# initc3/HoneyBadgerMPC

Measured on AMD Instinct MI355X. Metric: shares reconstructed/sec (batch open, n=64 t=21), higher is better.
Workload: dtype u256 (integer mod p): exact int8 x int8 -> int32 byte-split GEMM on the matrix cores; the high half of every sum folded mod p on the matrix cores too, one-word Barrett quotient

## Files before the change

### honeybadgermpc_amd/csrc/hb_mfma_fused.hip

```cpp
#include <math.h>

#include <algorithm>
#include <atomic>
#include <type_traits>

#include "hb_mm8.hpp"

namespace hb {

#include "hb_mm8_body.inc"

constexpr int FS_WAVES = 8, FS_TPW = 4;
#ifdef HB_MM8_TIMING
__device__ unsigned long long g_fs_t[256 * 8 * 8];
#define FS_T(k) do { const unsigned long long tn_ = __builtin_amdgcn_s_memtime(); tacc[k] += tn_ - tlast; tlast = tn_; } while (0)
#else
#define FS_T(k) do { } while (0)
#endif
constexpr int FS_MAXD = 24, FS_MAXC = 104;
constexpr size_t FS_LDS_LIMIT = 156 * 1024;

struct FsIdx { uint16_t z[FS_MAXD], xz[FS_MAXD], zc[FS_MAXC], xzc[FS_MAXC]; };
struct FsPick { const uint4 *cand; const uint32_t *cand_crow; int n_coef, nc; uint16_t zc[FS_MAXC]; };
struct FsSplit { uint32_t terms[FS_WAVES]; };
struct FsPack { int nm, ns; uint8_t single[8]; };
__host__ __device__ inline int fs_slot(const FsPack &pk, int i, int n_out, int &kind) {
    kind = 0;
    if (!(pk.nm | pk.ns)) return i;
    const int base = 16 * ((n_out + 15) / 16 - 1);
    int before = 0;
    for (int k = 0; k < pk.ns; k++) {
        if (pk.single[k] == i) { kind = 2; return base + 4 + (k & 3) + 8 * (k >> 2); }
        before += pk.single[k] < i;
    }
    const int pos = i - before;
    if (pos >= base) kind = 1;
    return pos;
}
static bool fs_pack_decide(int d, int n_coef, int nc, const uint8_t *small, FsPack *pk) {
    memset(pk, 0, sizeof *pk);
    const int n_out = n_coef + nc, rem = n_out - 16 * ((n_out + 15) / 16 - 1);
    if ((int64_t)d * 8 * 128 * 128 > MM8_BIAS_PACK) return false;
    if (rem <= 8) { pk->nm = rem; return true; }
    if (rem == 16) return false;
    int ns = 0;
    for (int i = n_coef - 1; i >= 0 && ns < 8; i--)
        if (small[i]) pk->single[ns++] = (uint8_t)i;
    std::reverse(pk->single, pk->single + ns);
    if (rem - ns > 4) { memset(pk, 0, sizeof *pk); return false; }
    pk->nm = rem - ns; pk->ns = ns;
    return true;
}
constexpr int FS_CAND_MAXN = 128;

__host__ __device__ inline int fs_ms_q(int d) { return (d + 1) * 64 + d * 8; }
__host__ __device__ inline size_t fs_lds_bytes(int n_rt, int nkb, int ms_d = 0) {
    return ((size_t)n_rt * 64 + (size_t)n_rt * nkb * 2 * 64 + (size_t)2 * FS_TPW * nkb * 4 * 64 + MM8_FOLD_Q + (ms_d ? fs_ms_q(ms_d) : 0)) * 16 +
           (size_t)(32 + 16 * n_rt) * 4;
}

#define FS_REDUCE(I_, F_, E_, C0_) \
    do { \
        const int i = (I_); \
        const int md = maskl[i]; \
        const bool live = chunk < n_chunks; \
        const bool cmp = live && md > 0, st = live && md < 0; \
        uint32_t ew[8]; \
        load_words<8>(ew, in_pk + (cmp ? (chunk * in_sc + (int64_t)(md - 1) * in_sl) * 8 : 0)); \
        uint64_t pw[8]; \
        { \
            const uint4 *cr = reinterpret_cast<const uint4 *>(crl + (size_t)i * 16); \
        _Pragma("unroll") \
            for (int k = 0; k < 4; k++) { \
                const uint4 c = cr[k]; \
                pw[2 * k] = (uint64_t)c.x | ((uint64_t)c.y << 32); \
                pw[2 * k + 1] = (uint64_t)c.z | ((uint64_t)c.w << 32); \
            } \
        } \
        uint32_t glo[5], ghi[5]; \
        _Pragma("unroll") \
        for (int k = 0; k < 12; k++) { \
            uint64_t gk = (uint64_t)F_(k) * k256 + (k < 7 ? pw[k] : 0ull); \
            if (k < 11) gk += (uint64_t)E_(k) * k16m; \
            if (k < 7) pw[k] = gk; \
            else { glo[k - 7] = (uint32_t)gk; ghi[k - 7] = (uint32_t)(gk >> 32); } \
        } \
        pw[0] += (uint64_t)(C0_) * u1; \
        pw[7] += (uint64_t)glo[0] * u1; \
        uint32_t hw[5]; \
        { \
            unsigned cyw = 0; \
        _Pragma("unroll") \
            for (int k = 0; k < 4; k++) hw[k] = __builtin_addc(glo[k + 1], ghi[k], cyw, &cyw); \
            hw[4] = ghi[4] + cyw; \
        } \
        v4i hb; \
        _Pragma("unroll") \
        for (int k = 0; k < 4; k++) hb[k] = (int)(hw[k] ^ 0x80808080u); \
        v4i dcol[8]; \
        _Pragma("unroll") \
        for (int eb = 0; eb < 8; eb++) \
            dcol[eb] = __builtin_amdgcn_mfma_i32_16x16x64_i8(fold_lane[eb * (MM8_FOLD_ROW / 16)], hb, v4i{0, 0, 0, 0}, 0, 0, 0); \
        _Pragma("unroll") \
        for (int k = 0; k < 8; k++) pw[k] += (uint64_t)hw[4] * bp.c384[k]; \
        _Pragma("unroll") \
        for (int k = 0; k < 8; k++) { \
            int64_t tt = (int64_t)pw[k] + (int64_t)dcol[k][0] * s1; \
            tt += (int64_t)dcol[k][1] * s256; \
            tt += (int64_t)dcol[k][2] * s64k; \
            tt += (int64_t)dcol[k][3] * s16m; \
            pw[k] = (uint64_t)tt; \
        } \
        const uint64_t tq = pw[7] + (pw[6] >> 32); \
        const uint32_t qh = (uint32_t)(((uint64_t)(uint32_t)(tq >> 16) * bp.mu) >> 46); \
        _Pragma("unroll") \
        for (int k = 0; k < 8; k++) pw[k] += (uint64_t)qh * bp.pneg[k]; \
        uint32_t ow[8]; \
        uint32_t top; \
        { \
            unsigned cy = 0; \
            ow[0] = (uint32_t)pw[0]; \
        _Pragma("unroll") \
            for (int k = 1; k < 8; k++) ow[k] = __builtin_addc((uint32_t)pw[k], (uint32_t)(pw[k - 1] >> 32), cy, &cy); \
            top = (uint32_t)(pw[7] >> 32) + cy - qh; \
        } \
        if (__builtin_amdgcn_ballot_w64(top != 0 || ow[7] >= ~bp.pneg[7]) != 0) { \
            uint32_t u[8]; \
            unsigned cy2 = 0; \
        _Pragma("unroll") \
            for (int k = 0; k < 8; k++) u[k] = __builtin_addc(ow[k], bp.pneg[k], cy2, &cy2); \
            const bool take = cy2 || top; \
        _Pragma("unroll") \
            for (int k = 0; k < 8; k++) ow[k] = take ? u[k] : ow[k]; \
        } \
        uint32_t diff = 0; \
        _Pragma("unroll") \
        for (int k = 0; k < 8; k++) diff |= ew[k] ^ ow[k]; \
        asm volatile("" : "+v"(diff), "+v"(ow[0]), "+v"(ow[1]), "+v"(ow[2]), "+v"(ow[3]), "+v"(ow[4]), "+v"(ow[5]), "+v"(ow[6]), "+v"(ow[7])); \
        const unsigned long long bad_lanes = __builtin_amdgcn_ballot_w64(cmp && diff); \
        if (bad_lanes) { \
            const uint32_t bits16 = (uint32_t)((bad_lanes | (bad_lanes >> 16) | (bad_lanes >> 32) | (bad_lanes >> 48)) & 0xffffull); \
            if (lane == 0) { \
                const int64_t tile_base = chunk - n; \
                const int32_t cmin = (int32_t)tile_base + __builtin_ctz(bits16); \
                if (*reinterpret_cast<volatile int32_t *>(mismatch) == 0) atomicOr(mismatch, 1); \
                if (first_bad && *reinterpret_cast<volatile int32_t *>(first_bad) > cmin) atomicMin(first_bad, cmin); \
                if (bad_map) atomicOr(bad_map + (tile_base >> 5), bits16 << (tile_base & 31)); \
            } \
        } \
        const int64_t oidx = chunk * out_sc + (int64_t)(-md - 1) * out_sl; \
        if (st && oidx < out_count) store_words<8>(out_pk + oidx * 8, ow); \
    } while (0)

template <int NKB, int PK, bool MSC>
__global__ __launch_bounds__(64 * FS_WAVES, 2) void k_mm8f(const int4 *__restrict__ a8, const uint32_t *__restrict__ crowd, const v4i *__restrict__ foldg,
                                                          const uint32_t *__restrict__ KT, const PrescaleParams PP,
                                                          const uint32_t *__restrict__ in_pk, int64_t in_sc, int64_t in_sl, const int32_t *__restrict__ in_rows,
                                                          int64_t in_count, int d, const int32_t *__restrict__ rowmode,
                                                          uint32_t *__restrict__ out_pk, int64_t out_sc, int64_t out_sl, int64_t out_count,
                                                          int32_t *__restrict__ mismatch, int32_t *__restrict__ first_bad, uint32_t *__restrict__ bad_map,
                                                          int n_out, int n_rt, int64_t n_chunks, int64_t n_units, BarrettParams bp, const FsDone done, const FsPick pick,
                                                          const FsSplit split, const v4i *__restrict__ MS) {
    constexpr bool PACKED = PK != 0;
    const int n_slots = PACKED ? 16 * n_rt : n_out;
    constexpr int NT = 64 * FS_WAVES, NL = 9, NW = 8;
    extern __shared__ uint4 fs_lds[];
    const int lane = threadIdx.x & 63, wave = __builtin_amdgcn_readfirstlane(threadIdx.x >> 6);
    const int n = lane & 15, g = lane >> 4;
    uint32_t *crl = reinterpret_cast<uint32_t *>(fs_lds);
    int4 *abuf = reinterpret_cast<int4 *>(fs_lds + n_rt * 64);
    uint4 *xbuf = fs_lds + n_rt * 64 + n_rt * NKB * 2 * 64;
    constexpr int bufsz = FS_TPW * NKB * 4 * 64;
    int32_t *rowl = reinterpret_cast<int32_t *>(xbuf + 2 * bufsz);
    int32_t *maskl = rowl + 32;
    v4i *foldl = reinterpret_cast<v4i *>(maskl + 16 * n_rt);
    v4i *msl = foldl + MM8_FOLD_Q;

#ifdef HB_MM8_TIMING
    unsigned long long tacc[8] = {0, 0, 0, 0, 0, 0, 0, 0}, tlast = __builtin_amdgcn_s_memtime();
#endif
    auto unit_chunk = [&](int64_t unit) {
        const int64_t chunk = unit * 64 + lane;
        return chunk >= n_chunks ? n_chunks - 1 : chunk;
    };
    auto fetch_row = [&](int64_t chunk, int row, uint32_t (&w)[NW], bool &okk) {
        const int64_t idx = chunk * in_sc + (int64_t)row * in_sl;
        okk = idx < in_count;
        load_words<NW>(w, in_pk + (okk ? idx : 0) * NW);
    };
    const uint32_t first_terms = (0x01010101u << wave) & (d < 32 ? (1u << d) - 1u : ~0u);
    uint32_t x_first[NW] = {0, 0, 0, 0, 0, 0, 0, 0};
    bool ok_first = false;
    if (first_terms) {
        const int l0 = __builtin_ctz(first_terms);
        fetch_row(unit_chunk(blockIdx.x), in_rows ? in_rows[l0] : l0, x_first, ok_first);
    }
    uint4 pk_piece = make_uint4(0, 0, 0, 0), pk_crow = make_uint4(0, 0, 0, 0);
    const int pk_e = threadIdx.x;
    const bool pk_has_piece = !PACKED && pick.cand && pk_e < pick.nc * NKB * 8, pk_has_crow = !PACKED && pick.cand && pk_e < pick.nc * 4;
    if (pk_has_piece) {
        const int j = pk_e / (NKB * 8), pc = pk_e - j * (NKB * 8);
        pk_piece = pick.cand[(size_t)pick.zc[j] * (NKB * 8) + pc];
    }
    if (pk_has_crow) pk_crow = reinterpret_cast<const uint4 *>(pick.cand_crow)[(size_t)pick.zc[pk_e >> 2] * 4 + (pk_e & 3)];
    {
        const int tid = threadIdx.x, n_mask = n_rt * 16, n_crow = n_rt * 64, n_img = n_rt * NKB * 2 * 64;
        const int lc = tid < d ? tid : d - 1;
        int32_t rw = in_rows ? in_rows[lc] : lc;
        int32_t mk = rowmode[tid < n_slots ? tid : 0];
        v4i cr = reinterpret_cast<const v4i *>(crowd)[tid < n_crow ? tid : 0];
        v4i fo = foldg[tid < MM8_FOLD_Q ? tid : 0];
        v4i img[3];
#pragma unroll
        for (int k = 0; k < 3; k++) img[k] = reinterpret_cast<const v4i *>(a8)[tid + k * NT < n_img ? tid + k * NT : 0];
        const int n_ms = MSC ? fs_ms_q(d) : 0;
        v4i msv[4];
        if constexpr (MSC) {
#pragma unroll
            for (int k = 0; k < 4; k++) msv[k] = MS[tid + k * NT < n_ms ? tid + k * NT : 0];
        }
        asm volatile("" : "+v"(rw), "+v"(mk), "+v"(cr), "+v"(fo), "+v"(img[0]), "+v"(img[1]), "+v"(img[2]));
        if constexpr (MSC) asm volatile("" : "+v"(msv[0]), "+v"(msv[1]), "+v"(msv[2]), "+v"(msv[3]));
        if (tid < 32) rowl[tid] = rw;
        if (tid < n_mask) maskl[tid] = tid < n_slots ? mk : 0;
        if (tid < n_crow) reinterpret_cast<v4i *>(fs_lds)[tid] = cr;
        if (tid < MM8_FOLD_Q) foldl[tid] = fo;
#pragma unroll
        for (int k = 0; k < 3; k++)
            if (tid + k * NT < n_img) reinterpret_cast<v4i *>(abuf)[tid + k * NT] = img[k];
        if constexpr (MSC) {
#pragma unroll
            for (int k = 0; k < 4; k++)
                if (tid + k * NT < n_ms) msl[tid + k * NT] = msv[k];
        }
        for (int i = tid + NT; i < n_mask; i += NT) maskl[i] = i < n_slots ? rowmode[i] : 0;
        for (int i = tid + NT; i < n_crow; i += NT) fs_lds[i] = reinterpret_cast<const uint4 *>(crowd)[i];
        for (int i = tid + 3 * NT; i < n_img; i += NT) abuf[i] = a8[i];
        if constexpr (MSC)
            for (int i = tid + 4 * NT; i < n_ms; i += NT) msl[i] = MS[i];
    }
    for (int i = threadIdx.x; i < (8 * NKB - d) * 256; i += NT) {
        const int l = d + (i >> 8), b = (i >> 7) & 1, t = (i >> 5) & 3, h = (i >> 4) & 1, c = i & 15;
        const int kb = l >> 3, gg = (l & 7) >> 1, e = l & 1;
        xbuf[(size_t)b * bufsz + (size_t)((((t * NKB + kb) * 2 + e) * 2 + h) * 64) + (c + 16 * gg)] = make_uint4(0, 0, 0, 0);
    }
    const int n_pairs = FS_TPW * n_rt;
    const uint32_t my_terms = (uint32_t)__builtin_amdgcn_readfirstlane((int)split.terms[wave]);

    uint32_t ms64k = 1u << 16;
    if constexpr (MSC) asm volatile("" : "+s"(ms64k));
    auto scale_unit = [&](auto first, int64_t unit, uint4 *dst, uint32_t terms) {
        constexpr bool FIRST = decltype(first)::value;
        const int64_t chunk = unit_chunk(unit);
        const int t = lane >> 4;
        uint32_t xw[NW];
        bool ok = false;
        auto fetch = [&](int l, uint32_t (&w)[NW], bool &okk) { fetch_row(chunk, FIRST ? (in_rows ? in_rows[l] : l) : rowl[l], w, okk); };
        terms &= d < 32 ? (1u << d) - 1u : ~0u;
        int l = terms ? __builtin_ctz(terms) : d;
        if constexpr (FIRST) {
#pragma unroll
            for (int k = 0; k < NW; k++) xw[k] = x_first[k];
            ok = ok_first;
        } else if (l < d) fetch(l, xw, ok);
        while (l < d) {
            terms &= terms - 1u;
            const int ln = terms ? __builtin_ctz(terms) : d;
            uint32_t xn[NW];
            bool okn = false;
            fetch(ln < d ? ln : l, xn, okn);
            uint32_t w[NW];
            bool over;
            if constexpr (MSC) {
                const v4i *tab;
                if constexpr (FIRST) tab = MS; else tab = msl;
                const v4i *al = tab + (g == (n >> 2) ? l * 64 + (n & 3) : d * 64);
                const v4i *cl = tab + (d + 1) * 64 + l * 8;
                const v4i b0 = v4i{(int)(xw[0] ^ 0x80808080u), (int)(xw[1] ^ 0x80808080u), (int)(xw[2] ^ 0x80808080u), (int)(xw[3] ^ 0x80808080u)};
                const v4i b1 = v4i{(int)(xw[4] ^ 0x80808080u), (int)(xw[5] ^ 0x80808080u), (int)(xw[6] ^ 0x80808080u), (int)(xw[7] ^ 0x80808080u)};
                v4i mc[8];
#pragma unroll
                for (int eb = 0; eb < 8; eb++) mc[eb] = __builtin_amdgcn_mfma_i32_16x16x64_i8(al[eb * 4], b0, cl[eb], 0, 0, 0);
#pragma unroll
                for (int eb = 0; eb < 8; eb++) mc[eb] = __builtin_amdgcn_mfma_i32_16x16x64_i8(al[32 + eb * 4], b1, mc[eb], 0, 0, 0);
                uint64_t mw[8];
#pragma unroll
                for (int k = 0; k < 8; k++) {
                    const uint32_t lo = (uint32_t)mc[k][0] + ((uint32_t)mc[k][1] << 8), hi = (uint32_t)mc[k][2] + ((uint32_t)mc[k][3] << 8);
                    mw[k] = (uint64_t)hi * ms64k + lo;
                }
                const uint64_t tq = mw[7] + (mw[6] >> 32);
                const uint32_t mq = (uint32_t)(((uint64_t)(uint32_t)(tq >> 16) * bp.mu) >> 46);
#pragma unroll
                for (int k = 0; k < 8; k++) mw[k] += (uint64_t)mq * bp.pneg[k];
                unsigned cyw = 0;
                w[0] = (uint32_t)mw[0];
#pragma unroll
                for (int k = 1; k < 8; k++) w[k] = __builtin_addc((uint32_t)mw[k], (uint32_t)(mw[k - 1] >> 32), cyw, &cyw);
                over = (uint32_t)(mw[7] >> 32) + cyw != mq;
            } else {
                const uint32_t *__restrict__ T = KT + (size_t)l * (NL * NL);
                uint32_t xd[NL];
                unpack<NL, NW>(xd, xw);
                uint64_t col[NL + 1];
#pragma unroll
                for (int j = 0; j <= NL; j++) col[j] = 0;
#pragma unroll
                for (int q = 0; q < NL; q++)
#pragma unroll
                    for (int j = 0; j < NL; j++) col[j] += (uint64_t)xd[q] * T[q * NL + j];
                uint32_t v[NL + 1];
#pragma unroll
                for (int k = 0; k < NL; k++) { v[k] = (uint32_t)col[k] & DMASK; col[k + 1] += col[k] >> LB; }
                v[NL] = (uint32_t)col[NL];
                const uint64_t mid = (uint64_t)v[9] * PP.m0 + (uint64_t)v[8] * PP.m1 + (((uint64_t)v[8] * PP.m0) >> LB);
                const uint64_t qh = (uint64_t)v[9] * PP.m1 + (mid >> LB);
                const uint32_t q0 = (uint32_t)qh & DMASK, q1 = (uint32_t)(qh >> LB);
                uint64_t dc[NL];
#pragma unroll
                for (int k = 0; k < NL; k++) {
                    dc[k] = v[k] + (uint64_t)q0 * PP.pbar[k];
                    if (k > 0) dc[k] += (uint64_t)q1 * PP.pbar[k - 1];
                }
                uint32_t r[NL];
#pragma unroll
                for (int k = 0; k < NL; k++) {
                    r[k] = (uint32_t)dc[k] & DMASK;
                    if (k < NL - 1) dc[k + 1] += dc[k] >> LB;
                }
                pack<NL, NW>(w, r);
                over = (r[NL - 1] >> 24) != 0;
            }
            const uint32_t *pneg = MSC ? bp.pneg : PP.pneg;
            if (pneg[NW - 1] >> 31) {
#pragma unroll
                for (int k = 0; k < NW; k++) w[k] = ok ? w[k] : 0u;
            } else {
                uint32_t u[NW];
                unsigned cy = 0;
#pragma unroll
                for (int k = 0; k < NW; k++) u[k] = __builtin_addc(w[k], pneg[k], cy, &cy);
                const bool take = cy || over;
#pragma unroll
                for (int k = 0; k < NW; k++) w[k] = ok ? (take ? u[k] : w[k]) : 0u;
            }
            const int kb = l >> 3, gg = (l & 7) >> 1, e = l & 1;
            uint4 *slot = dst + (size_t)(((t * NKB + kb) * 2 + e) * 2) * 64 + (n + 16 * gg);
            slot[0] = make_uint4(w[0], w[1], w[2], w[3]);
            slot[64] = make_uint4(w[4], w[5], w[6], w[7]);
#pragma unroll
            for (int k = 0; k < NW; k++) xw[k] = xn[k];
            ok = okn;
            l = ln;
        }
    };

    scale_unit(std::true_type{}, blockIdx.x, xbuf, first_terms);
    if (!PACKED && pick.cand) {
        __syncthreads();
        auto put = [&](int e, const uint4 &v) {
            const int j = e / (NKB * 8), pc = e - j * (NKB * 8);
            const int ri = pick.n_coef + j, rt = ri >> 4, r16 = ri & 15, r = 4 * (r16 & 3) + (r16 >> 2);
            const int kb = pc >> 3, grp = (pc >> 2) & 1, gg = pc & 3;
            reinterpret_cast<uint4 *>(abuf)[((rt * NKB + kb) * 2 + grp) * 64 + r + 16 * gg] = v;
        };
        if (pk_has_piece) put(pk_e, pk_piece);
        for (int e = pk_e + NT; e < pick.nc * NKB * 8; e += NT) {
            const int j = e / (NKB * 8), pc = e - j * (NKB * 8);
            put(e, pick.cand[(size_t)pick.zc[j] * (NKB * 8) + pc]);
        }
        if (pk_has_crow) fs_lds[(pick.n_coef + (pk_e >> 2)) * 4 + (pk_e & 3)] = pk_crow;
        for (int j = threadIdx.x; j < pick.nc; j += NT) maskl[pick.n_coef + j] = (int32_t)pick.zc[j] + 1;
    }

    const v4i biasv = v4i{MM8_BIAS, MM8_BIAS, MM8_BIAS, MM8_BIAS};
    uint32_t k256 = 256u, k16m = 1u << 24;
    int32_t s1 = 1, s256 = 256, s64k = 1 << 16, s16m = 1 << 24;
    uint32_t u1 = 1u;
    asm volatile("" : "+s"(k256), "+s"(k16m), "+s"(s1), "+s"(s256), "+s"(s64k), "+s"(s16m), "+s"(u1));
    const v4i *fold_lane = reinterpret_cast<const v4i *>(reinterpret_cast<const char *>(foldl) + (g == (n >> 2) ? 16 * n : 256));

    int buf = 0;
    int64_t unit = blockIdx.x;
    FS_T(0);
    for (; unit < n_units; unit += gridDim.x, buf ^= 1) {
        asm volatile("s_waitcnt lgkmcnt(0)" ::: "memory");
        FS_T(7);
        __builtin_amdgcn_s_barrier();
        FS_T(1);
        if (my_terms && unit + gridDim.x < n_units) scale_unit(std::false_type{}, unit + gridDim.x, xbuf + (size_t)(buf ^ 1) * bufsz, my_terms);
        FS_T(2);
        for (int pidx = wave; pidx < n_pairs; pidx += FS_WAVES) {
            const int tl = n_rt == 2 ? (pidx >> 1) : pidx / n_rt;
            const int rt = n_rt == 2 ? ((pidx ^ (pidx >> 2)) & 1) : pidx - tl * n_rt;
            const int64_t chunk = (unit * FS_TPW + tl) * 16 + n;
            const uint4 *xs = xbuf + (size_t)buf * bufsz + (size_t)tl * NKB * 4 * 64 + lane;
            const int4 *as = abuf + (size_t)rt * NKB * 2 * 64 + lane;
            uint32_t eap[4][11], c0p[4];
            const int rows_here = n_out - 16 * rt < 16 ? n_out - 16 * rt : 16;
            const int nreg = PACKED ? 4 : (rows_here + 3) >> 2;
            const uint32_t xs_addr = (uint32_t)(uintptr_t)(__attribute__((address_space(3))) const void *)xs;
            const uint32_t as_addr = (uint32_t)(uintptr_t)(__attribute__((address_space(3))) const void *)as;
            if (PACKED && rt == n_rt - 1) {
                const v4i biaspv = v4i{MM8_BIAS_PACK, MM8_BIAS_PACK, MM8_BIAS_PACK, MM8_BIAS_PACK};
                auto park_merged = [&](auto rc, const v4i (&acc)[20]) __attribute__((always_inline)) {
                    constexpr int r = decltype(rc)::value;
                    c0p[r] = (uint32_t)acc[0][r];
#pragma unroll
                    for (int j = 0; j < 11; j++) {
                        uint32_t lo = 0, hi = 0;
                        if (j < 9) { lo = (uint32_t)acc[1 + 2 * j][r]; hi = (uint32_t)acc[2 + 2 * j][r]; }
                        if (j >= 2) { lo += (uint32_t)acc[2 * j - 3][r + 2]; hi += (uint32_t)acc[2 * j - 2][r + 2]; }
                        if (j == 1) hi += (uint32_t)acc[0][r + 2];
                        eap[r][j] = lo + (hi << 8);
                    }
                };
                auto park_single = [&](auto rc, const v4i (&acc)[20]) __attribute__((always_inline)) {
                    constexpr int r = decltype(rc)::value;
                    c0p[r] = (uint32_t)acc[0][r];
#pragma unroll
                    for (int j = 0; j < 11; j++) eap[r][j] = j < 9 ? (uint32_t)acc[1 + 2 * j][r] + ((uint32_t)acc[2 + 2 * j][r] << 8) : 0u;
                };
                auto keep = [&](auto rc) __attribute__((always_inline)) {
                    constexpr int r = decltype(rc)::value;
                    asm volatile("" ::"v"(c0p[r]), "v"(eap[r][0]), "v"(eap[r][1]), "v"(eap[r][2]), "v"(eap[r][3]), "v"(eap[r][4]), "v"(eap[r][5]),
                                 "v"(eap[r][6]), "v"(eap[r][7]), "v"(eap[r][8]), "v"(eap[r][9]), "v"(eap[r][10]));
                    __builtin_amdgcn_sched_barrier(0);
                };
                {
                    v4i acc[20];
                    asm volatile("" ::: "memory");
                    __builtin_amdgcn_sched_barrier(0);
                    __builtin_amdgcn_s_setprio(0);
                    Mm8PhasePacked<NKB, 0>::run(acc, xs_addr, as_addr, biaspv);
                    __builtin_amdgcn_s_setprio(2);
                    __builtin_amdgcn_sched_barrier(0);
                    FS_T(3);
                    park_merged(std::integral_constant<int, 0>{}, acc);
                    keep(std::integral_constant<int, 0>{});
                    if constexpr (PK == 1) park_merged(std::integral_constant<int, 1>{}, acc);
                    else park_single(std::integral_constant<int, 1>{}, acc);
                    keep(std::integral_constant<int, 1>{});
                    if constexpr (PK == 2) {
                        park_single(std::integral_constant<int, 3>{}, acc);
                        keep(std::integral_constant<int, 3>{});
                    }
                }
                {
                    v4i acc[20];
                    asm volatile("" ::: "memory");
                    __builtin_amdgcn_sched_barrier(0);
                    FS_T(4);
                    __builtin_amdgcn_s_setprio(0);
                    Mm8PhasePacked<NKB, 1>::run(acc, xs_addr, as_addr, biaspv);
                    __builtin_amdgcn_s_setprio(2);
                    __builtin_amdgcn_sched_barrier(0);
                    FS_T(5);
                    auto pair_merged = [&](auto rc, int k) __attribute__((always_inline)) {
                        constexpr int r = decltype(rc)::value;
                        uint32_t lo = 0, hi = 0;
                        if (k < 10) { lo = (uint32_t)acc[2 * k][r]; hi = (uint32_t)acc[2 * k + 1][r]; }
                        if (k >= 2) { lo += (uint32_t)acc[2 * k - 4][r + 2]; hi += (uint32_t)acc[2 * k - 3][r + 2]; }
                        return lo + (hi << 8);
                    };
                    auto pair_single = [&](auto rc, int k) __attribute__((always_inline)) {
                        constexpr int r = decltype(rc)::value;
                        return k < 10 ? (uint32_t)acc[2 * k][r] + ((uint32_t)acc[2 * k + 1][r] << 8) : 0u;
                    };
#define FS_FM0(k) pair_merged(std::integral_constant<int, 0>{}, k)
#define FS_FM1(k) pair_merged(std::integral_constant<int, 1>{}, k)
#define FS_FS1(k) pair_single(std::integral_constant<int, 1>{}, k)
#define FS_FS3(k) pair_single(std::integral_constant<int, 3>{}, k)
#define FS_E0(k) eap[0][k]
#define FS_E1(k) eap[1][k]
#define FS_E3(k) eap[3][k]
                    if constexpr (PK == 2) { FS_REDUCE(16 * rt + 12 + g, FS_FS3, FS_E3, c0p[3]); __builtin_amdgcn_sched_barrier(0); }
                    FS_REDUCE(16 * rt + g, FS_FM0, FS_E0, c0p[0]);
                    if constexpr (PK == 1) FS_REDUCE(16 * rt + 4 + g, FS_FM1, FS_E1, c0p[1]);
                    else FS_REDUCE(16 * rt + 4 + g, FS_FS1, FS_E1, c0p[1]);
#undef FS_FM0
#undef FS_FM1
#undef FS_FS1
#undef FS_FS3
#undef FS_E0
#undef FS_E1
#undef FS_E3
                }
                FS_T(6);
                continue;
            }
            {
                v4i acc[24];
                asm volatile("" ::: "memory");
                __builtin_amdgcn_sched_barrier(0);
                __builtin_amdgcn_s_setprio(0);
                Mm8Phase<NKB, 0, false>::run(acc, xs_addr, as_addr, biasv);
                __builtin_amdgcn_s_setprio(2);
                __builtin_amdgcn_sched_barrier(0);
                FS_T(3);
#pragma unroll
                for (int reg = 0; reg < 4; reg++) {
                    if (reg >= 2 && reg >= nreg) break;
                    c0p[reg] = (uint32_t)acc[0][reg];
#pragma unroll
                    for (int j = 0; j < 11; j++) eap[reg][j] = (uint32_t)acc[1 + 2 * j][reg] + ((uint32_t)acc[2 + 2 * j][reg] << 8);
                    asm volatile("" ::"v"(c0p[reg]), "v"(eap[reg][0]), "v"(eap[reg][1]), "v"(eap[reg][2]), "v"(eap[reg][3]), "v"(eap[reg][4]),
                                 "v"(eap[reg][5]), "v"(eap[reg][6]), "v"(eap[reg][7]), "v"(eap[reg][8]), "v"(eap[reg][9]), "v"(eap[reg][10]));
                    __builtin_amdgcn_sched_barrier(0);
                }
            }
            {
                v4i acc[24];
                asm volatile("" ::: "memory");
                __builtin_amdgcn_sched_barrier(0);
                FS_T(4);
                __builtin_amdgcn_s_setprio(0);
                Mm8Phase<NKB, 1, false>::run(acc, xs_addr, as_addr, biasv);
                __builtin_amdgcn_s_setprio(2);
                __builtin_amdgcn_sched_barrier(0);
                FS_T(5);
#pragma unroll
                for (int reg = 0; reg < 4; reg++) {
                    if (reg >= 2 && reg >= nreg) break;
#define FS_F(k) ((uint32_t)acc[2 * (k)][reg] + ((uint32_t)acc[2 * (k) + 1][reg] << 8))
#define FS_E(k) eap[reg][k]
                    FS_REDUCE(16 * rt + 4 * reg + g, FS_F, FS_E, c0p[reg]);
#undef FS_F
#undef FS_E
                    if (reg & 1) __builtin_amdgcn_sched_barrier(0);
                }
            }
            FS_T(6);
        }
    }
#ifdef HB_MM8_TIMING
    if (lane == 0 && blockIdx.x < 256) for (int k = 0; k < 8; k++) g_fs_t[(blockIdx.x * 8 + wave) * 8 + k] = tacc[k];
#endif
    fs_workgroup_done(done, mismatch, first_bad);
}

typedef __int128 i128;

struct FsConsts {
    uint32_t c80r[9], biasmod[9], biasmod_pm[9], biasmod_ps[9];
    uint32_t ms_c80[9], ms_bias[9], pneg[8];
};
constexpr int FS_MS_BIAS = 1 << 20;
constexpr int32_t FS_OVERFLOW = 0x40000000;

__device__ __forceinline__ size_t fs_digit_addr(int i, int l, int b, int nkb) {
    const int lane_ = (4 * ((i % 16) % 4) + (i % 16) / 4) + 16 * ((l % 8) / 2), el = l & 1;
    const int grp = b >> 3, r7 = 7 - (b & 7), hi = r7 >> 2, bi = r7 & 3;
    return ((((size_t)(i / 16) * nkb + l / 8) * 2 + grp) * 64 + (size_t)lane_) * 16 + 4 * (2 * hi + el) + bi;
}

__device__ __forceinline__ void fs_row_constant(const FpParams<9> &P, const FsConsts &cs, const i128 *row, int d, uint32_t *dst16, int kind = 0) {
    constexpr int NL = 9, NW = 8;
    uint32_t s5[5] = {0, 0, 0, 0, 0};
    for (int l = 0; l < d; l++) {
        const i128 v = row[l];
        const uint32_t vw[5] = {(uint32_t)v, (uint32_t)(v >> 32), (uint32_t)(v >> 64), (uint32_t)(v >> 96), (uint32_t)(v >> 127 >> 1)};
        unsigned cy = 0;
#pragma unroll
        for (int k = 0; k < 5; k++) s5[k] = __builtin_addc(s5[k], vw[k], cy, &cy);
    }
    const bool negs = (s5[4] >> 31) != 0;
    if (negs) {
        unsigned cy = 1;
#pragma unroll
        for (int k = 0; k < 5; k++) s5[k] = __builtin_addc(~s5[k], 0u, cy, &cy);
    }
    uint32_t w8[NW] = {s5[0], s5[1], s5[2], s5[3], s5[4], 0, 0, 0}, fe[NL], prod[NL], corr[NL], k80[NL], bm[NL];
    unpack<NL, NW>(fe, w8);
    if (negs) fp_neg(fe, fe, P);
#pragma unroll
    for (int k = 0; k < NL; k++) { k80[k] = cs.c80r[k]; bm[k] = kind == 0 ? cs.biasmod[k] : kind == 1 ? cs.biasmod_pm[k] : cs.biasmod_ps[k]; }
    mont_mul(prod, fe, k80, P);
    fp_sub(corr, prod, bm, P);
    uint32_t cw[NW];
    pack<NL, NW>(cw, corr);
#pragma unroll
    for (int k = 0; k < 8; k++) {
        const uint64_t pair = (uint64_t)cw[k] + ((0x1010ull << 32) | 0x10100000ull);
        dst16[2 * k] = (uint32_t)pair;
        dst16[2 * k + 1] = (uint32_t)(pair >> 32);
    }
}

__device__ __forceinline__ void fs_build_body(uint8_t *fb_lds, const FpParams<9> &P, const uint32_t *__restrict__ inv, int n, const FsIdx &ix, int d, int nc, int n_coef,
                                              int flags, const FsConsts &cs, uint8_t *__restrict__ a8, uint32_t *__restrict__ crow, uint32_t *__restrict__ KT,
                                              int32_t *__restrict__ rowmode, int32_t *__restrict__ z_dev, int32_t *__restrict__ status, const FsPack &pk,
                                              uint8_t *__restrict__ ms = nullptr) {
    constexpr int NL = 9, NW = 8;
    const int n_out = n_coef + nc, nkb = (d + 7) / 8, n_rt = (n_out + 15) / 16;
    i128 *ent = reinterpret_cast<i128 *>(fb_lds);
    i128 *Ac = ent + (size_t)n_out * d;
    uint32_t *wj = reinterpret_cast<uint32_t *>(Ac + (d + 1));
    uint32_t *part = wj + (size_t)d * NL;
    const int tid = threadIdx.x;
    const bool do_z = flags & FS_BUILD_Z, do_zc = flags & FS_BUILD_ZC;
    if (do_z) {
        const size_t img = (size_t)n_rt * nkb * 2 * 64 * 16;
        for (size_t i = tid; i < img / 16; i += 1024) reinterpret_cast<uint4 *>(a8)[i] = make_uint4(0, 0, 0, 0);
        for (int i = tid; i < n_rt * 16 * 8; i += 1024) { crow[2 * i] = 0x10100000u; crow[2 * i + 1] = 0x1010u; }
        for (int i = tid; i < n_rt * 16; i += 1024) rowmode[i] = 0;
        if (tid < d) z_dev[tid] = ix.z[tid];
    }
    if (do_z && tid < 64) {
        if (tid <= d) Ac[tid] = tid == 0 ? 1 : 0;
        __builtin_amdgcn_fence(__ATOMIC_RELEASE, "wavefront");
        __builtin_amdgcn_wave_barrier();
        for (int q = 0; q < d; q++) {
            i128 nv = 0;
            const bool act = tid <= q + 1 && tid <= d;
            if (act) nv = (tid > 0 ? Ac[tid - 1] : (i128)0) - (i128)ix.xz[q] * Ac[tid];
            __builtin_amdgcn_fence(__ATOMIC_ACQ_REL, "wavefront");
            __builtin_amdgcn_wave_barrier();
            if (act) Ac[tid] = nv;
            __builtin_amdgcn_fence(__ATOMIC_ACQ_REL, "wavefront");
            __builtin_amdgcn_wave_barrier();
        }
        if (tid < d) {
            const i128 xj = ix.xz[tid];
            i128 cur = 1;
            for (int m = d - 1; m >= 0; m--) {
                if (m < n_coef) ent[(size_t)m * d + tid] = cur;
                if (m > 0) cur = Ac[m] + xj * cur;
            }
        }
    } else if (do_z && tid < 64 + 4 * FS_MAXD + 32) {
        const int j = (tid - 64) >> 2, pq = (tid - 64) & 3;
        if (j < d) {
            uint32_t w[NL];
            fp_set(w, P.one);
            const uint32_t *row = inv + (size_t)ix.z[j] * n * NL;
            for (int q = pq; q < d; q += 4) {
                if (q == j) continue;
                uint32_t f[NL];
#pragma unroll
                for (int k = 0; k < NL; k++) f[k] = row[(size_t)ix.z[q] * NL + k];
                mont_mul(w, w, f, P);
            }
#pragma unroll
            for (int k = 0; k < NL; k++) part[((size_t)j * 4 + pq) * NL + k] = w[k];
        }
    } else if (do_zc && tid >= 256) {
        for (int e = tid - 256; e < nc * d; e += 1024 - 256) {
            const int i = e / d, j = e - i * d;
            const int64_t xi = ix.xzc[i];
            i128 v = 1;
            for (int q = 0; q < d; q++)
                if (q != j) v *= (i128)(xi - (int64_t)ix.xz[q]);
            ent[(size_t)(n_coef + i) * d + j] = v;
        }
    }
    __syncthreads();
    if (do_z && tid < d) {
        uint32_t a[NL], b[NL], c[NL];
#pragma unroll
        for (int k = 0; k < NL; k++) { a[k] = part[((size_t)tid * 4) * NL + k]; b[k] = part[((size_t)tid * 4 + 1) * NL + k]; }
// ... 418 lines not shown
```

Before: 9.481 billion.

## Prefetch all first-unit rows and software-pipeline their matrix-core scaling from LDS

For the MSC path, the prologue now loads every row this wave needs for the first unit up front, and stages only the per-wave slices of the scaling table into LDS instead of the whole table. The first unit is then processed by a dedicated block that overlaps the MFMA products of row j with the Barrett fold and store of row j-1, with sched barriers between stages. It also picks a non-canonical path when the modulus allows it, which skips the final conditional subtract. The aim is to hide global-load latency and MFMA latency in the startup phase, at the cost of more registers for the prefetched rows and accumulators.

```diff
diff --git a/honeybadgermpc_amd/csrc/hb_mfma_fused.hip b/honeybadgermpc_amd/csrc/hb_mfma_fused.hip
--- a/honeybadgermpc_amd/csrc/hb_mfma_fused.hip
+++ b/honeybadgermpc_amd/csrc/hb_mfma_fused.hip
@@ -191,7 +191,9 @@
     const uint32_t first_terms = (0x01010101u << wave) & (d < 32 ? (1u << d) - 1u : ~0u);
     uint32_t x_first[NW] = {0, 0, 0, 0, 0, 0, 0, 0};
     bool ok_first = false;
-    if (first_terms) {
+    uint32_t xf[MSC ? NKB : 1][NW];
+    bool okf[MSC ? NKB : 1];
+    if (!MSC && first_terms) {
         const int l0 = __builtin_ctz(first_terms);
         fetch_row(unit_chunk(blockIdx.x), in_rows ? in_rows[l0] : l0, x_first, ok_first);
     }
@@ -213,14 +215,28 @@
         v4i img[3];
 #pragma unroll
         for (int k = 0; k < 3; k++) img[k] = reinterpret_cast<const v4i *>(a8)[tid + k * NT < n_img ? tid + k * NT : 0];
-        const int n_ms = MSC ? fs_ms_q(d) : 0;
-        v4i msv[4];
+        const int ms_lj = wave + 8 * (lane >> 3), ms_cq = (d + 1) * 64 + (ms_lj < d ? ms_lj : d - 1) * 8 + (lane & 7);
+        v4i msv[MSC ? NKB + 1 : 1];
         if constexpr (MSC) {
 #pragma unroll
-            for (int k = 0; k < 4; k++) msv[k] = MS[tid + k * NT < n_ms ? tid + k * NT : 0];
+            for (int j = 0; j < NKB; j++) {
+                const int l = wave + 8 * j, lc = l < d ? l : d - 1;
+                msv[j] = MS[lc * 64 + lane];
+            }
+            msv[NKB] = MS[ms_cq];
+            const int64_t chunk0 = unit_chunk(blockIdx.x);
+#pragma unroll
+            for (int j = 0; j < NKB; j++) {
+                const int l = wave + 8 * j, lc = l < d ? l : d - 1;
+                fetch_row(chunk0, in_rows ? in_rows[lc] : lc, xf[j], okf[j]);
+                okf[j] = okf[j] && l < d;
+            }
         }
         asm volatile("" : "+v"(rw), "+v"(mk), "+v"(cr), "+v"(fo), "+v"(img[0]), "+v"(img[1]), "+v"(img[2]));
-        if constexpr (MSC) asm volatile("" : "+v"(msv[0]), "+v"(msv[1]), "+v"(msv[2]), "+v"(msv[3]));
+        if constexpr (MSC) {
+#pragma unroll
+            for (int j = 0; j <= NKB; j++) asm volatile("" : "+v"(msv[j]));
+        }
         if (tid < 32) rowl[tid] = rw;
         if (tid < n_mask) maskl[tid] = tid < n_slots ? mk : 0;
         if (tid < n_crow) reinterpret_cast<v4i *>(fs_lds)[tid] = cr;
@@ -230,14 +246,16 @@
             if (tid + k * NT < n_img) reinterpret_cast<v4i *>(abuf)[tid + k * NT] = img[k];
         if constexpr (MSC) {
 #pragma unroll
-            for (int k = 0; k < 4; k++)
-                if (tid + k * NT < n_ms) msl[tid + k * NT] = msv[k];
+            for (int j = 0; j < NKB; j++) {
+                const int l = wave + 8 * j, lc = l < d ? l : d - 1;
+                msl[lc * 64 + lane] = msv[j];
+            }
+            if (lane < 8 * NKB) msl[ms_cq] = msv[NKB];
+            msl[d * 64 + lane] = v4i{0, 0, 0, 0};
         }
         for (int i = tid + NT; i < n_mask; i += NT) maskl[i] = i < n_slots ? rowmode[i] : 0;
         for (int i = tid + NT; i < n_crow; i += NT) fs_lds[i] = reinterpret_cast<const uint4 *>(crowd)[i];
         for (int i = tid + 3 * NT; i < n_img; i += NT) abuf[i] = a8[i];
-        if constexpr (MSC)
-            for (int i = tid + 4 * NT; i < n_ms; i += NT) msl[i] = MS[i];
     }
     for (int i = threadIdx.x; i < (8 * NKB - d) * 256; i += NT) {
         const int l = d + (i >> 8), b = (i >> 7) & 1, t = (i >> 5) & 3, h = (i >> 4) & 1, c = i & 15;
@@ -272,8 +290,8 @@
             uint32_t w[NW];
             bool over;
             if constexpr (MSC) {
-                const v4i *tab;
-                if constexpr (FIRST) tab = MS; else tab = msl;
+                static_assert(!FIRST, "the first unit's matrix-core tasks are the block at the call site");
+                const v4i *tab = msl;
                 const v4i *al = tab + (g == (n >> 2) ? l * 64 + (n & 3) : d * 64);
                 const v4i *cl = tab + (d + 1) * 64 + l * 8;
                 const v4i b0 = v4i{(int)(xw[0] ^ 0x80808080u), (int)(xw[1] ^ 0x80808080u), (int)(xw[2] ^ 0x80808080u), (int)(xw[3] ^ 0x80808080u)};
@@ -355,7 +373,67 @@
         }
     };
 
-    scale_unit(std::true_type{}, blockIdx.x, xbuf, first_terms);
+    if constexpr (MSC) {
+        const int t = lane >> 4;
+        const bool diag = g == (n >> 2);
+        auto first_block = [&](auto canon_c) __attribute__((always_inline)) {
+            constexpr bool CANON = decltype(canon_c)::value;
+            v4i mc[NKB][8];
+#pragma unroll
+            for (int s = 0; s <= NKB; s++) {
+                if (s < NKB) {
+                    const int j = s, l = wave + 8 * j, lc = l < d ? l : d - 1;
+                    const v4i *al = msl + (diag ? lc * 64 + (n & 3) : d * 64);
+                    const v4i *cl = msl + (d + 1) * 64 + lc * 8;
+                    const v4i b0 = v4i{(int)(xf[j][0] ^ 0x80808080u), (int)(xf[j][1] ^ 0x80808080u), (int)(xf[j][2] ^ 0x80808080u), (int)(xf[j][3] ^ 0x80808080u)};
+                    const v4i b1 = v4i{(int)(xf[j][4] ^ 0x80808080u), (int)(xf[j][5] ^ 0x80808080u), (int)(xf[j][6] ^ 0x80808080u), (int)(xf[j][7] ^ 0x80808080u)};
+#pragma unroll
+                    for (int eb = 0; eb < 8; eb++) mc[j][eb] = __builtin_amdgcn_mfma_i32_16x16x64_i8(al[eb * 4], b0, cl[eb], 0, 0, 0);
+#pragma unroll
+                    for (int eb = 0; eb < 8; eb++) mc[j][eb] = __builtin_amdgcn_mfma_i32_16x16x64_i8(al[32 + eb * 4], b1, mc[j][eb], 0, 0, 0);
+                }
+                if (s > 0) {
+                    const int j = s - 1, l = wave + 8 * j;
+                    uint64_t mw[8];
+#pragma unroll
+                    for (int k = 0; k < 8; k++) {
+                        const uint32_t lo = (uint32_t)mc[j][k][0] + ((uint32_t)mc[j][k][1] << 8), hi = (uint32_t)mc[j][k][2] + ((uint32_t)mc[j][k][3] << 8);
+                        mw[k] = (uint64_t)hi * ms64k + lo;
+                    }
+                    const uint64_t tq = mw[7] + (mw[6] >> 32);
+                    const uint32_t mq = (uint32_t)(((uint64_t)(uint32_t)(tq >> 16) * bp.mu) >> 46);
+#pragma unroll
+                    for (int k = 0; k < 8; k++) mw[k] += (uint64_t)mq * bp.pneg[k];
+                    uint32_t w[NW];
+                    unsigned cyw = 0;
+                    w[0] = (uint32_t)mw[0];
+#pragma unroll
+                    for (int k = 1; k < 8; k++) w[k] = __builtin_addc((uint32_t)mw[k], (uint32_t)(mw[k - 1] >> 32), cyw, &cyw);
+                    if constexpr (CANON) {
+                        const bool over = (uint32_t)(mw[7] >> 32) + cyw != mq;
+                        uint32_t u[NW];
+                        unsigned cy = 0;
+#pragma unroll
+                        for (int k = 0; k < NW; k++) u[k] = __builtin_addc(w[k], bp.pneg[k], cy, &cy);
+                        const bool take = cy || over;
+#pragma unroll
+                        for (int k = 0; k < NW; k++) w[k] = okf[j] ? (take ? u[k] : w[k]) : 0u;
+                    } else {
+#pragma unroll
+                        for (int k = 0; k < NW; k++) w[k] = okf[j] ? w[k] : 0u;
+                    }
+                    const int gg = (l & 7) >> 1, e = l & 1;
+                    uint4 *slot = xbuf + (size_t)(((t * NKB + j) * 2 + e) * 2) * 64 + (n + 16 * gg);
+                    slot[0] = make_uint4(w[0], w[1], w[2], w[3]);
+                    slot[64] = make_uint4(w[4], w[5], w[6], w[7]);
+                }
+                __builtin_amdgcn_sched_barrier(0);
+            }
+        };
+        if (bp.pneg[NW - 1] >> 31) first_block(std::false_type{});
+        else first_block(std::true_type{});
+    } else
+        scale_unit(std::true_type{}, blockIdx.x, xbuf, first_terms);
     if (!PACKED && pick.cand) {
         __syncthreads();
         auto put = [&](int e, const uint4 &v) {
```

New measurement: 9.671 billion (median of 6 runs). 1.02x the previous value.
